# jwr1995/Conv-TasNet

Measured on AMD Instinct MI355X. Metric: utterances/sec (4s, 8kHz, 2-spk) fwd+bwd, higher is better.
Workload: dtype bf16; 1 GPU; paper config train step c2: N=256 L=20 B=256 H=512 P=3 X=8 R=4 gLN non-causal relu-mask, 2 spk, 4 s @ 8 kHz, fwd+PIT loss+bwd+clip+Adam; per_gpu_batch=32, global_batch=32, samples=32000, frames=3199, parallelism=dp1, hip_graph=False

## Files before the change

### conv-tasnet_amd/csrc/ctn_capi.hip

```cpp
#include <stdlib.h>
#include <math.h>
#include <stdarg.h>
#include <stdio.h>
#include <string.h>

#include <atomic>
#include <mutex>
#include <string>
#include <vector>

#include "../../include/ctn.h"
#include "ctn_common.h"
#include "ctn_kernels.h"

using namespace ctn;

static thread_local char g_err[512] = "";

static int fail(int code, const char* fmt, ...) __attribute__((format(printf, 2, 3)));
static int fail(int code, const char* fmt, ...) {
  va_list ap;
  va_start(ap, fmt);
  vsnprintf(g_err, sizeof(g_err), fmt, ap);
  va_end(ap);
// ... 162 lines not shown
  int dev = 0;
  if (hipGetDevice(&dev) != hipSuccess || dev < 0 || dev >= MAX_DEV) return CTN_OK;
  const uint32_t* h = g_deverr.mirror[dev].load(std::memory_order_acquire);
  if (!h) return CTN_OK;
  const uint32_t w = *(const volatile uint32_t*)h;
  if (w) return fail(CTN_ERR_HIP, "device error word 0x%x: %s", w, dev_err_text(w));
  return CTN_OK;
}

hipError_t dev_err_refresh(hipStream_t s) {
  int dev = 0;
  uint32_t* w = dev_err_word(&dev);
  volatile uint32_t* h = w ? dev_err_mirror(dev) : nullptr;
  if (!h) return hipErrorOutOfMemory;
  return hipMemcpyAsync((void*)h, w, 4, hipMemcpyDeviceToHost, s);
}
}

uint32_t* ctn::device_error_word() {
  int dev = 0;
  return dev_err_word(&dev);
}

extern "C" int ctn_device_status(void* stream, uint32_t* word, int clear) {
  int dev = 0;
  uint32_t* dw = dev_err_word(&dev);
  volatile uint32_t* mirror = dw ? dev_err_mirror(dev) : nullptr;
  if (!mirror) return fail(CTN_ERR_HIP, "device error word: unavailable");
  hipStream_t s = (hipStream_t)stream;
  uint32_t w = 0;
// ... 111 lines not shown
  return g;
}
GemmRows tb_gemmB(const ctn_tblock_desc* d, bool fused) {
  GemmRows g{};
  g.g = Rows{d->M, d->K, d->Kp};
  g.Kred = d->H; g.Nout = d->B; g.norm = d->norm_type;
  g.lda = d->H; g.ldw = d->H; g.epi = EPI_RESID; g.ldr = d->B; g.ldc = d->B;
  if (fused) {
    g.aop.kind = OP_NORM1_BWD; g.aop.norm = d->norm_type;
  }
  return g;
}
static int ws_fold_mask() {
  const char* e = getenv("CTN_WS_FOLD");
  return e ? atoi(e) : 3;
}

bool tb_fused_n1(const ctn_tblock_desc* d) {
  const char* e = getenv("CTN_FUSE_N1");
  if (e && atoi(e) == 0) return false;
  if (d->dtype != CTN_DTYPE_BF16 || (d->norm_type != CTN_NORM_GLN && d->norm_type != CTN_NORM_CLN)) return false;
  if (gemm_dual_eligible(BF16, tb_dualB(d))) return false;
  GemmRows g = tb_gemmB(d, true);
  static const float dummy[2] = {0.f, 0.f};
  g.aop.aux = dummy; g.aop.apart = const_cast<float*>(dummy); g.aop.aout = const_cast<float*>(dummy);
  g.aop.stats = reinterpret_cast<const float2*>(dummy); g.aop.sums = reinterpret_cast<const float2*>(dummy);
  return gemm_ws_eligible(BF16, g);
}
DType tb_dt(const ctn_tblock_desc* d) { return d->dtype == CTN_DTYPE_BF16 ? BF16 : F32; }

// ... 324 lines not shown
    w1 = L.w1s;
    w2 = L.w2s;
  }
  GemmRows g1 = tb_gemm1(d);
  g1.A = x;
  g1.W = w1;
  g1.Wf = w1f;
  g1.alpha = p->alpha1;
  g1.C = sv->h1;
  g1.grp_slab = L.slab1;
  const bool fin1 = d->norm_type == CTN_NORM_CLN && gemm_ws_final_cln(dt, g1);
  if (fin1) {
    g1.stats_out = st1;
    g1.eps = (float)kEps;
  }
  {
    TimedScope ts(CTN_TIMER_GEMM1, s);
    CTN_HIP(launch_gemm_rows(dt, g1, s));
  }
  const bool fold = d->norm_type == CTN_NORM_GLN;
  if (!fold && !fin1) CTN_HIP(launch_stats_finalize(L.slab1, G, L.parts1, cnt, 0, (float)kEps, st1, s));
  DwArgs da{};
  da.g = rg; da.H = d->H; da.P = d->P; da.dil = d->dilation; da.pad = tb_pad(d); da.norm = d->norm_type;
  da.seg = dw_seg(da, false);
  da.h1 = sv->h1; da.st1 = st1;
  da.alpha1 = p->alpha1; da.gamma1 = p->gamma1; da.beta1 = p->beta1; da.alpha2 = p->alpha2;
  da.wd = p->wd; da.d_out = sv->d; da.slab2 = L.slab2;
  if (fold) da.f_st1 = gemm_rows_stat_fold(dt, g1, L.slab1, cnt, (float)kEps, 0, st1);
  if (d->norm_type == CTN_NORM_CLN) {
    da.st2_out = st2;
    da.eps = (float)kEps;
  }
  {
    TimedScope ts(CTN_TIMER_DW_FWD, s);
    CTN_HIP(launch_dw_fwd(dt, da, s));
  }
  GemmRows g2{};
  g2.g = rg; g2.Kred = d->H; g2.Nout = d->B; g2.norm = d->norm_type;
  g2.A = sv->d; g2.lda = d->H;
  g2.aop.kind = OP_PRELU_NORM; g2.aop.norm = d->norm_type; g2.aop.stats = st2;
  g2.aop.gamma = p->gamma2; g2.aop.beta = p->beta2; g2.aop.alpha = p->alpha2;
  g2.W = w2; g2.ldw = d->H; g2.Wf = w2f;
  g2.epi = EPI_RESID; g2.R = x; g2.ldr = d->B;
// ... 99 lines not shown
  GemmRows ga = tb_gemmA(d);
  ga.A = gy;
  ga.W = w2t;
  ga.Wf = w2tf;
  ga.R = sv->d;
  ga.alpha = p->alpha2; ga.stats = st2; ga.gamma = p->gamma2;
  ga.C = L.G1;
  ga.grp_slab = L.slabA;
  GemmDual duA = tb_dualA(d);
  duA.A = gy; duA.W = w2t; duA.Wf = w2tf; duA.R = sv->d; duA.C = L.G1;
  duA.alpha = p->alpha2; duA.stats = st2; duA.gamma = p->gamma2; duA.grp_slab = L.slabA;
  duA.Bm = sv->d;
  duA.bop.stats = st2; duA.bop.gamma = p->gamma2; duA.bop.beta = p->beta2; duA.bop.alpha = p->alpha2;
  duA.Dpart = L.cpart2;
  const bool dualA = gemm_dual_eligible(dt, duA);
  if (dualA) {
    TimedScope ts(CTN_TIMER_GEMM_A, s);
    CTN_HIP(launch_gemm_dual(duA, s));
  } else {
    {
      TimedScope ts(CTN_TIMER_GEMM_A, s);
      CTN_HIP(launch_gemm_rows(dt, ga, s));
    }
    GemmCols c2{};
    c2.g = rg; c2.P = d->B; c2.Q = d->H;
    c2.A = gy; c2.lda = d->B;
    c2.B = sv->d; c2.ldb = d->H;
    c2.bop.kind = OP_PRELU_NORM; c2.bop.norm = d->norm_type; c2.bop.stats = st2;
    c2.bop.gamma = p->gamma2; c2.bop.beta = p->beta2; c2.bop.alpha = p->alpha2;
    c2.Cpart = L.cpart2; c2.nchunks = L.chunks2;
    CTN_HIP(launch_gemm_cols(dt, c2, s));
  }
  const bool fold = d->norm_type == CTN_NORM_GLN;

  DwArgs da{};
  da.g = rg; da.H = d->H; da.P = d->P; da.dil = d->dilation; da.pad = tb_pad(d); da.norm = d->norm_type;
  da.seg = dw_seg(da, true);
  da.h1 = sv->h1; da.d = sv->d; da.st1 = st1; da.st2 = st2;
  da.alpha1 = p->alpha1; da.gamma1 = p->gamma1; da.beta1 = p->beta1; da.alpha2 = p->alpha2; da.gamma2 = p->gamma2;
  da.wd = p->wd;
  da.ga2 = L.G1; da.sm2 = L.sums2; da.ga1_out = L.G2; da.slab1 = L.slabD; da.col_slab = L.colD;
  if (fold)
    da.f_sm2 = dualA ? gemm_dual_stat_fold(duA, L.slabA, cnt, 0.f, 1, nullptr)
                     : gemm_rows_stat_fold(dt, ga, L.slabA, cnt, 0.f, 1, nullptr);
  else
    da.sm1_out = L.sums1;
  if (!fold) {
    if (dualA && L.partsA <= 4 && dw_wave_eligible(dt, da))
      da.f_sm2 = gemm_dual_stat_fold(duA, L.slabA, cnt, 0.f, 1, nullptr);
    else
      CTN_HIP(launch_stats_finalize(L.slabA, G, L.partsA, cnt, 1, 0.f, L.sums2, s));
  }
  {
    TimedScope ts(CTN_TIMER_DW_BWD, s);
    CTN_HIP(launch_dw_bwd(dt, da, s));
  }
  const bool fused1 = tb_fused_n1(d);
  int nalpha = ew_blocks(da);
  if (fused1) {
    GemmRows gb = tb_gemmB(d, true);
// ... 1108 lines not shown
```

### conv-tasnet_amd/csrc/ctn_common.h

```cpp
#pragma once
#include <hip/hip_runtime.h>
#include <stdint.h>

#include <type_traits>
#include <utility>

#define CTN_DEV __device__ __forceinline__

typedef uint16_t bf16raw;
struct alignas(16) u128 { uint32_t x, y, z, w; };

CTN_DEV float bf2f(uint16_t v) { return __uint_as_float(((uint32_t)v) << 16); }
CTN_DEV uint16_t f2bf(float f) { return __builtin_bit_cast(uint16_t, (__bf16)f); }

template <typename T> struct Vec8;

template <> struct Vec8<float> {
  static CTN_DEV void load(const float* p, float v[8]) {
    const float4 a = *reinterpret_cast<const float4*>(p);
    const float4 b = *reinterpret_cast<const float4*>(p + 4);
    v[0] = a.x; v[1] = a.y; v[2] = a.z; v[3] = a.w;
    v[4] = b.x; v[5] = b.y; v[6] = b.z; v[7] = b.w;
  }
  static CTN_DEV void store(float* p, const float v[8]) {
// ... 276 lines not shown
}

CTN_DEV float xsum_rows(float v) {
  auto q = __builtin_amdgcn_permlane16_swap(__float_as_uint(v), __float_as_uint(v), false, false);
  v = __uint_as_float(q[0]) + __uint_as_float(q[1]);
  auto r = __builtin_amdgcn_permlane32_swap(__float_as_uint(v), __float_as_uint(v), false, false);
  return __uint_as_float(r[0]) + __uint_as_float(r[1]);
}

template <int CTRL, int ROW_MASK> CTN_DEV double dpp_d(double x) {
  const unsigned long long b = __builtin_bit_cast(unsigned long long, x);
  const unsigned lo = (unsigned)__builtin_amdgcn_update_dpp(0, (int)(unsigned)b, CTRL, ROW_MASK, 0xF, false);
  const unsigned hi = (unsigned)__builtin_amdgcn_update_dpp(0, (int)(unsigned)(b >> 32), CTRL, ROW_MASK, 0xF, false);
  return __builtin_bit_cast(double, ((unsigned long long)hi << 32) | lo);
}
CTN_DEV double wave_sum_dpp_d(double v) {
  v += dpp_d<0xB1, 0xF>(v);
  v += dpp_d<0x4E, 0xF>(v);
  v += dpp_d<0x141, 0xF>(v);
  v += dpp_d<0x140, 0xF>(v);
  v += dpp_d<0x142, 0xA>(v);
  v += dpp_d<0x143, 0xC>(v);
  const unsigned long long b = __builtin_bit_cast(unsigned long long, v);
  const unsigned lo = (unsigned)__builtin_amdgcn_readlane((int)(unsigned)b, 63);
  const unsigned hi = (unsigned)__builtin_amdgcn_readlane((int)(unsigned)(b >> 32), 63);
  return __builtin_bit_cast(double, ((unsigned long long)hi << 32) | lo);
}

#ifndef CTN_IEEE_MAX
#define CTN_IEEE_MAX 0
// ... 48 lines not shown
__host__ __device__ inline int ws_runs_kmax(int ntile, int grid, int tpu) {
  const int twg = (ntile + grid - 1) / grid;
  return (twg + tpu - 1) / tpu + 1;
}

struct StatFold {
  const double2* slab = nullptr;
  int parts = 0;
  double cnt = 1.0;
  float eps = 0.f;
  int mode = 0;
  float2* out = nullptr;
  WsRuns ws;
};

CTN_DEV float2 fold_stat(const StatFold& f, int m) {
  double s = 0.0, ss = 0.0;
  const int lane = (int)(threadIdx.x & 63);
  if (f.ws.grid == 0) {
    const double2* sg = f.slab + (size_t)m * f.parts;
    for (int i = lane; i < f.parts; i += 256) {
      double2 v[4];
#pragma unroll
      for (int u = 0; u < 4; ++u) v[u] = i + 64 * u < f.parts ? sg[i + 64 * u] : make_double2(0.0, 0.0);
#pragma unroll
      for (int u = 0; u < 4; ++u)
        if (i + 64 * u < f.parts) {
          s += v[u].x;
          ss += v[u].y;
        }
    }
// ... 7 lines not shown
      return t0 < ws_t0(w, b + 1) ? f.slab[((size_t)b * w.waves + wv) * w.kmax + (m - t0 / w.tpu)]
                                  : make_double2(0.0, 0.0);
    };
    for (int i = lane; i < n; i += 256) {
      double2 v[4];
#pragma unroll
      for (int u = 0; u < 4; ++u) v[u] = i + 64 * u < n ? get(i + 64 * u) : make_double2(0.0, 0.0);
#pragma unroll
      for (int u = 0; u < 4; ++u)
        if (i + 64 * u < n) {
          s += v[u].x;
          ss += v[u].y;
        }
    }
  }
  s = wave_sum(s);
  ss = wave_sum(ss);
  if (f.mode == 0) {
    const double mean = s / f.cnt;
    double var = ss / f.cnt - mean * mean;
    if (var < 0.0) var = 0.0;
    return make_float2((float)mean, (float)(1.0 / sqrt(var + (double)f.eps)));
  }
  return make_float2((float)(s / f.cnt), (float)(ss / f.cnt));
}

enum NormKind { NORM_GLN = 0, NORM_CLN = 1 };

template <int NK> CTN_DEV int stat_index(int row, int Kp) {
  return NK == NORM_GLN ? row / Kp : row;
}

static inline int ceil_div(long a, long b) { return (int)((a + b - 1) / b); }

template <class F, int... I> CTN_DEV void static_for_impl(F&& f, std::integer_sequence<int, I...>) {
  (f(std::integral_constant<int, I>{}), ...);
}
template <int N, class F> CTN_DEV void static_for(F&& f) { static_for_impl(f, std::make_integer_sequence<int, N>{}); }
```

### conv-tasnet_amd/csrc/ctn_dual_ws.hip

```cpp
#include <stdlib.h>

#include "ctn_common.h"
#include "ctn_kernels.h"

namespace ctn {

namespace {

typedef short bf16x8_t __attribute__((ext_vector_type(8)));
typedef short s16x4_t __attribute__((ext_vector_type(4)));
typedef float f32x4_t __attribute__((ext_vector_type(4)));

constexpr int DV_TM = 32;
#ifndef CTN_DV_NC
#define CTN_DV_NC 8
#endif
constexpr int DV_NR = 4, DV_NC = CTN_DV_NC, DV_NMW = 4;
static_assert(DV_NC == 4 || DV_NC == 8, "column waves");
constexpr int DV_ND = DV_NR + DV_NC;
constexpr int DV_NT = (DV_ND + DV_NMW) * 64;
constexpr int DV_KB = 8, DV_KR = 256;
constexpr int DV_NS = 128;
constexpr int DV_GRID = 256;
#ifndef CTN_DV_RAWB
// ... 167 lines not shown

template <int NK, int NSL, int PF, bool COLS = false>
__global__ __launch_bounds__(COLS ? (DV_NC + DV_NMW) * 64 : DV_NT) void gemm_dual_ws_kernel(GemmDual p) {
  constexpr int NR = COLS ? 0 : DV_NR;
  constexpr int ND = NR + DV_NC;
  constexpr int TM = DV_TM, KB = DV_KB, KR = DV_KR, NS = DV_NS;
  constexpr int SLOT = DV_SLOT;
  static_assert(NSL * SLOT <= 160 * 1024 - 2048, "LDS budget");
  __shared__ __attribute__((aligned(16))) char smem[NSL * SLOT];
  __shared__ __attribute__((aligned(16))) uint32_t fl_full[NSL][4];
  __shared__ __attribute__((aligned(16))) uint32_t fl_done[NSL][ND];
  __shared__ __attribute__((aligned(16))) float sgb[2][NS];
  constexpr bool CLNC = NK == NORM_CLN && !COLS && CTN_DV_CLNC;
  __shared__ __attribute__((aligned(16))) double2 cln_scr[CLNC ? 2 : 1][CLNC ? DV_NR * DV_TM : 1];
  __shared__ __attribute__((aligned(16))) uint32_t fl_rows[2][4];

  const int tid = threadIdx.x, lane = tid & 63, wid = __builtin_amdgcn_readfirstlane(tid >> 6);
  const int lr = lane & 15, lg = lane >> 4;
  const int S = p.Nout / NS;
  const int nr = (int)gridDim.x / S;
  int rr, sl;
  {
    const int b = (int)blockIdx.x;
    if ((int)gridDim.x % (8 * S) == 0) {
      const int l = b / 8;
      sl = l % S;
      rr = (b % 8) * (nr / 8) + l / S;
    } else {
      sl = b % S;
      rr = b / S;
    }
  }
  const long rows = p.g.rows();
  const int ntile = (int)(rows / TM);
  const int t0 = (int)((long)ntile * rr / nr), t1 = (int)((long)ntile * (rr + 1) / nr);
  const int n0 = sl * NS;
  const int Kp = p.g.Kp, Kv = p.g.K, tpu = Kp / TM;

  if (tid < NSL * 4) (&fl_full[0][0])[tid] = 0u;
  else if (tid < NSL * (4 + ND)) (&fl_done[0][0])[tid - NSL * 4] = 0u;
  else if (tid < NSL * (4 + ND) + 8) (&fl_rows[0][0])[tid - NSL * (4 + ND)] = 0u;
  if constexpr (!COLS)
    if (tid < 2 * NS) sgb[tid / NS][tid % NS] = (tid < NS ? p.bop.gamma : p.bop.beta)[n0 + tid % NS];
  __syncthreads();

  const float eal = COLS ? 0.f : p.alpha[0];
  const int kmax = ws_runs_kmax(ntile, nr, tpu);
  constexpr int COLS_LDT = KR + 4;
  static_assert(!COLS || NS * COLS_LDT * 4 <= NSL * DV_SLOT, "transpose image fits the ring");
  static_assert(!COLS || DV_RB, "COLS takes the raw-B slot layout (no operand transform)");
  auto store_tr = [&](float* Dp) __attribute__((always_inline)) {
    const float* img = reinterpret_cast<const float*>(smem);
    for (int idx = tid; idx < NS * (KR / 4); idx += (DV_NC + DV_NMW) * 64) {
      const int nl = idx / (KR / 4), k4 = idx % (KR / 4);
      *reinterpret_cast<float4*>(Dp + (size_t)(n0 + nl) * KR + 4 * k4) =
          *reinterpret_cast<const float4*>(img + nl * COLS_LDT + 4 * k4);
// ... 165 lines not shown
                p.grp_slab[((size_t)t * TM + 16 * rb + lr) * (S * DV_NR) + sl * DV_NR + r] = make_double2((double)s, (double)ss);
            }
          }
        }
        dv_signal(&fl_done[slot][r], gen);
        if (++slot == NSL) {
          slot = 0;
          ++gen;
        }
      }
      DV_ACC(3, tl0);
    };
    if (t0 < t1) {
      if (eal <= 1.f) run(std::true_type{});
      else run(std::false_type{});
      if constexpr (NK == NORM_GLN) flush();
    }
    DV_STAMP_STORE;
    return;
  }
  if (wid < ND) {
    dv_prio<2, NK>();
    constexpr int CJ = COLS ? DV_CJC : (DV_NI ? CTN_DV_CJN : DV_CJ), CI = 16 * (8 / CJ) / DV_NC;
    static_assert(CI >= 2 && CI <= 16 && CI % 2 == 0, "column split");
    const int c = wid - NR, wp = c / (8 / CJ), wn = c % (8 / CJ);
    DV_STAMP_DECL;
    f32x4_t dacc[CI][CJ];
#pragma unroll
    for (int i = 0; i < CI; ++i)
#pragma unroll
      for (int j = 0; j < CJ; ++j) dacc[i][j] = f32x4_t{0.f, 0.f, 0.f, 0.f};
// ... 355 lines not shown
```

### conv-tasnet_amd/csrc/ctn_dw_wave.hip

```cpp
#include <stdlib.h>

#include "ctn_common.h"
#include "ctn_dw.h"
#include "ctn_kernels.h"

namespace ctn {

namespace {

constexpr int WV_H = 512, WV_P = 3, WV_NB = 3;

struct WItem {
  int m, wgi, rho, j0, j1, base;
};
CTN_DEV WItem witem(const DwArgs& a, const CombGeom& gm) {
  const int wv = __builtin_amdgcn_readfirstlane((int)(threadIdx.x >> 6));
  WItem it;
  it.m = (int)blockIdx.x / gm.wgpu;
  it.wgi = (int)blockIdx.x % gm.wgpu;
  const int id = it.wgi * gm.ipw + wv;
  const bool active = id < gm.items;
  it.rho = active ? id / gm.nseg : 0;
  it.j0 = active ? (id % gm.nseg) * a.seg : 0;
  it.j1 = active ? min(it.j0 + a.seg, gm.jmax) : it.j0;
// ... 24 lines not shown

template <int NK, bool CAUSAL>
__global__ __launch_bounds__(256, 4) void dw_fwd_wave_kernel(DwArgs a) {
  constexpr int P = WV_P, H = WV_H;
  constexpr int POWN = CAUSAL ? P - 1 : (P - 1) / 2;
  constexpr int HT = P - 1 - POWN;
  __shared__ double red[16];
  const CombGeom gm = comb_geom(a);
  const WItem it = witem(a, gm);
  const int lane = threadIdx.x & 63;
  const int K = a.g.K, Kp = a.g.Kp, dil = a.dil;
  const long nbytes = a.g.rows() * H * 2;
  const rsrc_t rH = du_rsrc(a.h1, nbytes);
  const uint32_t vo = lane * 16;
  const float al1 = a.alpha1[0], al2 = a.alpha2[0];
  float2 st1u = make_float2(0.f, 0.f);
  if constexpr (NK == NORM_GLN) {
    const StatFold& f = a.f_st1;
    if (f.slab) {
      st1u = fold_stat(f, it.m);
      if (f.out && it.wgi == 0 && threadIdx.x == 0) f.out[it.m] = st1u;
    } else {
      st1u = a.st1[it.m];
    }
    st1u = uniform2(st1u);
  }
  float w[P][8], g1[8], b1[8];
#pragma unroll
  for (int e = 0; e < 8; ++e) {
    const int ch = lane * 8 + e;
    g1[e] = a.gamma1[ch];
    b1[e] = a.beta1[ch];
#pragma unroll
    for (int t = 0; t < P; ++t) w[t][e] = a.wd[ch * P + t];
  }
  const int jK = steps_below(K, it.rho, dil);
  auto row_at = [&](int s) { return it.base + ((unsigned)s < (unsigned)jK ? it.rho + s * dil : 0); };
  auto ld = [&](int row) {
    return __builtin_bit_cast(v4u, __builtin_amdgcn_raw_buffer_load_b128(rH, vo, row * (H * 2), (CTN_DW_NTL & 2) ? 2 : 0));
  };

  constexpr int CB = 63;
  float2 bst = make_float2(0.f, 0.f), nst = bst;
  int bbase = it.j0;
  auto batch_fetch = [&](int jb) { nst = a.st1[row_at(jb + lane + HT)]; };
  auto batch_next = [&]() {
    bbase += CB;
    bst = nst;
    batch_fetch(bbase + CB);
  };
  auto bcast = [&](float2 v, int j) {
    const int l = j - bbase;
    return make_float2(__int_as_float(__builtin_amdgcn_readlane(__float_as_int(v.x), l)),
                       __int_as_float(__builtin_amdgcn_readlane(__float_as_int(v.y), l)));
  };
// ... 2 lines not shown
    float x[8];
    unpack8(vh, x);
    const float nm = -st.x;
#pragma unroll
    for (int e = 0; e < 8; ++e) {
      const float ax = x[e] * al1;
      const float v = fmaf((sel_pos(x[e], x[e], ax) + nm) * st.y, g1[e], b1[e]);
      out[e] = EDGE ? (ok ? v : 0.f) : v;
    }
  };
  float win[3][8];
#pragma unroll
  for (int i = 0; i < P - 1; ++i) {
    const int sh = it.j0 - POWN + i;
    const int rh = row_at(sh);
    finish(std::true_type{}, ld(rh), (unsigned)sh < (unsigned)jK, NK == NORM_GLN ? st1u : a.st1[rh], win[i + 1]);
  }

  float ts = 0.f, tss = 0.f;
  RowPark pk;
  pk.j0 = it.j0;
  auto park_flush = [&](int n) {
    const int k = it.rho + (pk.j0 + lane) * dil;
    if (lane < n && k < Kp) {
      if (a.st2_out) {
        const double mean = (double)pk.s / H;
        double var = (double)pk.ss / H - mean * mean;
        if (var < 0.0) var = 0.0;
        a.st2_out[it.base + k] = make_float2((float)mean, (float)(1.0 / sqrt(var + (double)a.eps)));
      } else {
        a.slab2[it.base + k] = make_double2((double)pk.s, (double)pk.ss);
// ... 30 lines not shown
    } else {
      s = wave_sum_dpp(s);
      ss = wave_sum_dpp(ss);
      const int pq = j - pk.j0;
      pk.s = lane == pq ? s : pk.s;
      pk.ss = lane == pq ? ss : pk.ss;
    }
  };
  auto boundary = [&]() {
    park_flush(CB);
    pk.j0 = bbase + CB;
    batch_next();
  };

  const int jint = min(it.j1, jK - HT);
  v4u rb[WV_NB];
  if (it.j0 < it.j1) rb[0] = ld(row_at(it.j0 + HT));
  if (it.j0 + 1 < it.j1) rb[1] = ld(row_at(it.j0 + 1 + HT));
  if constexpr (NK != NORM_GLN) {
    batch_fetch(it.j0);
    bbase = it.j0 - CB;
    batch_next();
  }
  auto triple = [&](int jb) __attribute__((always_inline)) {
    static_for<3>([&](auto qc) __attribute__((always_inline)) {
      constexpr int q = decltype(qc)::value;
      const int j = jb + q;
      __builtin_amdgcn_sched_barrier(0);
      rb[(q + 2) % 3] = ld(row_at(j + 2 + HT));
      step(std::false_type{}, qc, j, rb[q]);
    });
  };
  int jb = it.j0;
// ... 40 lines not shown
  constexpr int GT = POWN;
  __shared__ double red[16];
  __shared__ float buf[256 * 8];
  const CombGeom gm = comb_geom(a);
  const WItem it = witem(a, gm);
  const int lane = threadIdx.x & 63;
  const int K = a.g.K, Kp = a.g.Kp, dil = a.dil;
  const long nbytes = a.g.rows() * H * 2;
  const rsrc_t rH = du_rsrc(a.h1, nbytes), rD = du_rsrc(a.d, nbytes), rG = du_rsrc(a.ga2, nbytes);
  const uint32_t vo = lane * 16;
  const float al1 = a.alpha1[0], al2 = a.alpha2[0];
  float2 st1u = make_float2(0.f, 0.f), st2u = st1u, sm2u = st1u;
  if constexpr (NK == NORM_GLN) {
    st1u = a.st1[it.m];
    st2u = a.st2[it.m];
    const StatFold& f = a.f_sm2;
    sm2u = f.slab ? fold_stat(f, it.m) : a.sm2[it.m];
    sm2u = uniform2(sm2u);
  }
  __shared__ __attribute__((aligned(16))) float cst[P + 3][H];
  for (int i = threadIdx.x; i < H; i += 256) {
    const int c = CTN_DW_CSTH ? ((i >> 2) & 1) * (H / 2) + (i >> 3) * 4 + (i & 3) : i;
#pragma unroll
    for (int t = 0; t < P; ++t) cst[t][c] = a.wd[i * P + t];
    cst[P][c] = a.gamma1[i];
    cst[P + 1][c] = a.beta1[i];
    cst[P + 2][c] = a.gamma2[i];
  }
  __syncthreads();
  auto cbase = [&]() __attribute__((always_inline)) {
    uint32_t b = lane * (CTN_DW_CSTH ? 16u : 32u);
    asm volatile("" : "+v"(b));
    return b;
  };
  auto cvec4 = [&](uint32_t b, int r, int hf) __attribute__((always_inline)) {
    return *reinterpret_cast<const float4*>(reinterpret_cast<const char*>(&cst[0][0]) + b + (r * H * 4 + hf * (CTN_DW_CSTH ? H * 2 : 16)));
  };
  auto f4 = [](const float4& v, int i) { return i == 0 ? v.x : i == 1 ? v.y : i == 2 ? v.z : v.w; };
  float cgam[8], cbet[8], cgam2[8], cbet2[8], cwd[P][8];
#pragma unroll
  for (int e = 0; e < 8; ++e) {
    cgam[e] = cbet[e] = cgam2[e] = cbet2[e] = 0.f;
#pragma unroll
    for (int t = 0; t < P; ++t) cwd[t][e] = 0.f;
// ... 98 lines not shown
    }
  };
  auto gstat = [&](int row, int j, bool batch, float2& st, float2& sm) __attribute__((always_inline)) {
    if constexpr (NK == NORM_GLN) {
      st = st2u;
      sm = sm2u;
    } else if (batch) {
      st = bcast(bst2, j);
      sm = bcast(bsm2, j);
    } else {
      st = a.st2[row];
      sm = sm_row(row);
    }
  };

#pragma unroll
  for (int i = 0; i < P - 1; ++i) {
    const int sg = it.j0 + GT - P + 1 + i;
    const int rg = row_at(sg);
    float2 st, sm;
    gstat(rg, 0, false, st, sm);
    finish_g(std::true_type{}, ld(rD, rg), ld(rG, rg), sg >= 0 && sg < jK, sg >= it.j0 && sg < it.j1, st, sm,
             gdw[i + 1]);
  }

  RowPark pk;
  pk.j0 = it.j0;
  auto park_flush = [&](int n) {
    const int k = it.rho + (pk.j0 + lane) * dil;
    if (lane < n && k < Kp) {
      if (a.sm1_out)
        a.sm1_out[it.base + k] = make_float2((float)((double)pk.s / H), (float)((double)pk.ss / H));
      else
        a.slab1[it.base + k] = make_double2((double)pk.s, (double)pk.ss);
    }
  };

// ... 55 lines not shown
    } else {
      s = wave_sum_dpp(s);
      ss = wave_sum_dpp(ss);
      const int pq = j - pk.j0;
      pk.s = lane == pq ? s : pk.s;
      pk.ss = lane == pq ? ss : pk.ss;
    }
  };
  auto boundary = [&]() {
    park_flush(CB);
    pk.j0 = bbase + CB;
    batch_next();
  };

  const int jint = min(it.j1, jK) - GT;
  BwdRow rb[WV_NB];
  if (it.j0 < it.j1) load_row(it.j0, rb[0]);
  if (it.j0 + 1 < it.j1) load_row(it.j0 + 1, rb[1]);
  if constexpr (NK != NORM_GLN) {
    batch_fetch(it.j0);
    bbase = it.j0 - CB;
    batch_next();
  }
  auto triple = [&](int jb) __attribute__((always_inline)) {
    static_for<3>([&](auto qc) __attribute__((always_inline)) {
      constexpr int q = decltype(qc)::value;
      const int j = jb + q;
      __builtin_amdgcn_sched_barrier(0);
      load_row(j + 2, rb[(q + 2) % 3]);
      step(std::false_type{}, qc, j, rb[q]);
    });
  };
  int jb = it.j0;
// ... 97 lines not shown
```

### conv-tasnet_amd/csrc/ctn_gemm_ws.hip

```cpp
#include <stdlib.h>

#include <type_traits>

#include "ctn_common.h"
#include "ctn_kernels.h"

namespace ctn {

typedef short bf16x8_t __attribute__((ext_vector_type(8)));
typedef float f32x4_t __attribute__((ext_vector_type(4)));

#ifndef CTN_WS_GRID
#define CTN_WS_GRID 256
#endif
constexpr int WS_WAVES = 8, WS_TM = 16, WS_GRID = CTN_WS_GRID;
#ifndef CTN_WS_DMA
#define CTN_WS_DMA 1
#endif
#ifndef CTN_WS_DR
#define CTN_WS_DR 6
#endif
constexpr int WS_DR = CTN_WS_DR;
#ifndef CTN_WS_FLAGS
#define CTN_WS_FLAGS 0
// ... 676 lines not shown
      if (t < t1) {
        step(t, accC, accP);
        epilogue(le1, t1 - 1, accC);
      } else {
        epilogue(le1, t1 - 1, accP);
      }
    }
  };
  const float al_any = (OPK == OP_PRELU_NORM || N1B) ? oal : eal;
  if constexpr (OPK == OP_PRELU_NORM || N1B || HAS_STATS) {
    if (al_any <= 1.f) run(std::true_type{});
    else run(std::false_type{});
  } else {
    run(std::true_type{});
  }
  if constexpr (HAS_STATS && NK == NORM_GLN) flush_run();
  if constexpr (CLN_FIN) {
    lds_barrier();
    cln_final(t1 - 1);
  }
#if CTN_WS_STAMP
  if (lane == 0)
    for (int i = 0; i < 8; ++i) ws_stamps[((size_t)blockIdx.x * 16 + wid) * 8 + i] = st_sum[i];
#endif
  if constexpr (N1B) {
    const float w = wave_sum_dpp(calpha);
    if (lane == 0) salpha[wid] = w;
    __syncthreads();
    if (tid == 0) {
      double a = 0.0;
      for (int i = 0; i < WV; ++i) a += (double)salpha[i];
// ... 94 lines not shown
static int ws_waves(const GemmRows& p) { return ws_wide(p) ? 16 * (p.Nout / 512) : 8; }
static int ws_tile_rows(const GemmRows& p) { return ws_wide(p) ? 32 : WS_TM; }
static int ws_slices(const GemmRows& p) { return p.Nout == 1536 ? 3 : ws_wide(p) ? CTN_WS_S512 : 1; }

template <int OPK, int NK, int EPI>
static hipError_t ws_launch_shape(const GemmRows& p, hipStream_t s) {
  int nb = 0, kb = 0;
  ws_shape(p.Nout, p.Kred, &nb, &kb);
  const dim3 grid(gemm_ws_grid(p));
  if (nb == 4 && kb == 8) {
    if constexpr (EPI == EPI_NORM_BWD)
      hipLaunchKernelGGL((gemm_ws_kernel<OPK, NK, EPI, 4, 8, 8, 1>), grid, dim3(512), 0, s, p);
    else if (ws_slices(p) == 3) {
      if constexpr (OPK == OP_PLAIN && EPI == EPI_STORE)
        hipLaunchKernelGGL((gemm_ws_kernel<OPK, NK, EPI, 2, 8, 16, 2, 3>), grid, dim3(1024), 0, s, p);
    } else if (ws_slices(p) == 2)
      hipLaunchKernelGGL((gemm_ws_kernel<OPK, NK, EPI, 2, 8, 8, 2, 2>), grid, dim3(512), 0, s, p);
    else
      hipLaunchKernelGGL((gemm_ws_kernel<OPK, NK, EPI, 2, 8, 16, 2>), grid, dim3(1024), 0, s, p);
  }
  else if (nb == 2 && kb == 16)
    hipLaunchKernelGGL((gemm_ws_kernel<OPK, NK, EPI, 2, 16, 8, 1>), grid, dim3(512), 0, s, p);
  else
    hipLaunchKernelGGL((gemm_ws_kernel<OPK, NK, EPI, 2, 8, 8, 1>), grid, dim3(512), 0, s, p);
  return hipGetLastError();
}

template <int NK>
static hipError_t ws_launch_nk(const GemmRows& p, hipStream_t s) {
  if (p.aop.kind == OP_PRELU_NORM) return ws_launch_shape<OP_PRELU_NORM, NK, EPI_RESID>(p, s);
// ... 19 lines not shown
```

### conv-tasnet_amd/csrc/ctn_kernels.h

```cpp
#pragma once
#include <hip/hip_runtime.h>
#include <stddef.h>
#include <stdint.h>

#include "ctn_common.h"

namespace ctn {

enum DType { F32 = 0, BF16 = 1 };

uint32_t* device_error_word();
enum RowOpKind { OP_PLAIN = 0, OP_NORM = 1, OP_PRELU_NORM = 2, OP_NORM1_BWD = 3 };
enum EpiKind { EPI_STORE = 0, EPI_PRELU_STATS = 1, EPI_RESID = 2, EPI_NORM_BWD = 3 };

struct RowOp {
  int kind = OP_PLAIN;
  int norm = 0;
  const float2* stats = nullptr;
  const float* gamma = nullptr;
  const float* beta = nullptr;
  const float* alpha = nullptr;
  StatFold fold;
  const void* aux = nullptr;
  const float2* sums = nullptr;
// ... 12 lines not shown
  const void* A; int lda;
  const void* W; int ldw;
  const void* Wf;
  RowOp aop;
  int epi = EPI_STORE;
  void* C; int ldc;
  const void* R = nullptr; int ldr = 0;
  const float* alpha = nullptr;
  const float2* stats = nullptr;
  const float* gamma = nullptr;
  int norm = 0;
  double2* grp_slab = nullptr;
  float2* stats_out = nullptr;
  float eps = 0.f;
  uint32_t* err = nullptr;
};
int gemm_rows_tiles_per_group(DType dt, const GemmRows& p);
hipError_t launch_gemm_rows(DType dt, const GemmRows& p, hipStream_t s);
bool gemm_ws_eligible(DType dt, const GemmRows& p);
int gemm_ws_grid(const GemmRows& p);
int gemm_ws_group_parts(const GemmRows& p);
WsRuns gemm_ws_runs(const GemmRows& p);
StatFold gemm_rows_stat_fold(DType dt, const GemmRows& p, const double2* slab, double cnt, float eps, int mode,
                             float2* out);
bool gemm_ws_can_fold(DType dt, const GemmRows& p);
bool gemm_ws_final_cln(DType dt, const GemmRows& p);
hipError_t launch_gemm_ws(const GemmRows& p, hipStream_t s);

struct GemmCols {
  Rows g;
// ... 12 lines not shown
  const void* A; int lda;
  const void* W; int ldw;
  const void* Wf;
  int epi = EPI_RESID;
  void* C; int ldc;
  const void* R = nullptr; int ldr = 0;
  const float* alpha = nullptr;
  const float2* stats = nullptr;
  const float* gamma = nullptr;
  int norm = 0;
  double2* grp_slab = nullptr;
  const void* Bm; int ldb;
  RowOp bop;
  float* Dpart;
  uint32_t* err = nullptr;
};
bool gemm_dual_eligible(DType dt, const GemmDual& p);
int gemm_dual_ranges(const GemmDual& p);
int gemm_dual_group_parts(const GemmDual& p);
int dual_ws_cln_parts_per_slice();
int dual_ws_row_waves(const GemmDual& p);
StatFold gemm_dual_stat_fold(const GemmDual& p, const double2* slab, double cnt, float eps, int mode,
                             float2* out);
hipError_t launch_gemm_dual(const GemmDual& p, hipStream_t s);
bool gemm_dual_ws_enabled();
bool gemm_dual_ws_eligible(const GemmDual& p);
int gemm_dual_ws_ranges(const GemmDual& p);
hipError_t launch_gemm_dual_ws(const GemmDual& p, hipStream_t s);
bool gemm_cols_ws_eligible(DType dt, const GemmCols& c);
int gemm_cols_ws_ranges(const GemmCols& c);
// ... 190 lines not shown
```

Baseline: 2401 utterances/sec.

## Add opt-in ticketed in-GEMM stat finalization and prefetch dw rows before stat fold

Result: no change. 2420 utterances/sec, median of 6 (+0.8%).

```diff
diff --git a/conv-tasnet_amd/csrc/ctn_capi.hip b/conv-tasnet_amd/csrc/ctn_capi.hip
--- a/conv-tasnet_amd/csrc/ctn_capi.hip
+++ b/conv-tasnet_amd/csrc/ctn_capi.hip
@@ -200,6 +200,34 @@
   volatile uint32_t* h = w ? dev_err_mirror(dev) : nullptr;
   if (!h) return hipErrorOutOfMemory;
   return hipMemcpyAsync((void*)h, w, 4, hipMemcpyDeviceToHost, s);
+}
+}
+
+constexpr uint32_t STAT_TICKETS = 1u << 15;
+__device__ uint32_t ctn_stat_ticket_words[STAT_TICKETS];
+
+namespace {
+struct StatTickets {
+  std::atomic<uint32_t*> base[MAX_DEV] = {};
+  std::atomic<uint32_t> next[MAX_DEV] = {};
+};
+StatTickets g_tickets;
+
+uint32_t* stat_tickets(int n) {
+  int dev = 0;
+  if (n < 1 || (uint32_t)n > STAT_TICKETS / 8) return nullptr;
+  if (hipGetDevice(&dev) != hipSuccess || dev < 0 || dev >= MAX_DEV) return nullptr;
+  uint32_t* b = g_tickets.base[dev].load(std::memory_order_acquire);
+  if (!b) {
+    void* a = nullptr;
+    if (hipGetSymbolAddress(&a, HIP_SYMBOL(ctn_stat_ticket_words)) != hipSuccess) return nullptr;
+    b = (uint32_t*)a;
+    g_tickets.base[dev].store(b, std::memory_order_release);
+  }
+  uint32_t o = g_tickets.next[dev].load(std::memory_order_relaxed), start;
+  do start = o + (uint32_t)n > STAT_TICKETS ? 0u : o;
+  while (!g_tickets.next[dev].compare_exchange_weak(o, start + (uint32_t)n, std::memory_order_relaxed));
+  return b + start;
 }
 }
 
@@ -341,6 +369,11 @@
 static int ws_fold_mask() {
   const char* e = getenv("CTN_WS_FOLD");
   return e ? atoi(e) : 3;
+}
+
+static bool stat_final_enabled() {
+  const char* e = getenv("CTN_STAT_FINAL");
+  return e && atoi(e) != 0;
 }
 
 bool tb_fused_n1(const ctn_tblock_desc* d) {
@@ -695,11 +728,18 @@
     g1.stats_out = st1;
     g1.eps = (float)kEps;
   }
+  const bool fold = d->norm_type == CTN_NORM_GLN;
+  bool final1 = false;
+  if (fold && stat_final_enabled() && gemm_ws_eligible(dt, g1)) {
+    g1.fin.f = gemm_rows_stat_fold(dt, g1, L.slab1, cnt, (float)kEps, 0, st1);
+    g1.fin.per_range = gemm_ws_grid(g1) / g1.fin.f.ws.grid;
+    g1.fin.ticket = stat_tickets(G);
+    final1 = g1.fin.ticket != nullptr;
+  }
   {
     TimedScope ts(CTN_TIMER_GEMM1, s);
     CTN_HIP(launch_gemm_rows(dt, g1, s));
   }
-  const bool fold = d->norm_type == CTN_NORM_GLN;
   if (!fold && !fin1) CTN_HIP(launch_stats_finalize(L.slab1, G, L.parts1, cnt, 0, (float)kEps, st1, s));
   DwArgs da{};
   da.g = rg; da.H = d->H; da.P = d->P; da.dil = d->dilation; da.pad = tb_pad(d); da.norm = d->norm_type;
@@ -707,7 +747,7 @@
   da.h1 = sv->h1; da.st1 = st1;
   da.alpha1 = p->alpha1; da.gamma1 = p->gamma1; da.beta1 = p->beta1; da.alpha2 = p->alpha2;
   da.wd = p->wd; da.d_out = sv->d; da.slab2 = L.slab2;
-  if (fold) da.f_st1 = gemm_rows_stat_fold(dt, g1, L.slab1, cnt, (float)kEps, 0, st1);
+  if (fold && !final1) da.f_st1 = gemm_rows_stat_fold(dt, g1, L.slab1, cnt, (float)kEps, 0, st1);
   if (d->norm_type == CTN_NORM_CLN) {
     da.st2_out = st2;
     da.eps = (float)kEps;
@@ -837,6 +877,13 @@
   duA.bop.stats = st2; duA.bop.gamma = p->gamma2; duA.bop.beta = p->beta2; duA.bop.alpha = p->alpha2;
   duA.Dpart = L.cpart2;
   const bool dualA = gemm_dual_eligible(dt, duA);
+  bool final2 = false;
+  if (dualA && d->norm_type == CTN_NORM_GLN && stat_final_enabled() && gemm_dual_ws_eligible(duA)) {
+    duA.fin.f = gemm_dual_stat_fold(duA, L.slabA, cnt, 0.f, 1, L.sums2);
+    duA.fin.per_range = duA.fin.f.ws.waves / dual_ws_row_waves(duA);
+    duA.fin.ticket = stat_tickets(G);
+    final2 = duA.fin.ticket != nullptr;
+  }
   if (dualA) {
     TimedScope ts(CTN_TIMER_GEMM_A, s);
     CTN_HIP(launch_gemm_dual(duA, s));
@@ -863,10 +910,10 @@
   da.alpha1 = p->alpha1; da.gamma1 = p->gamma1; da.beta1 = p->beta1; da.alpha2 = p->alpha2; da.gamma2 = p->gamma2;
   da.wd = p->wd;
   da.ga2 = L.G1; da.sm2 = L.sums2; da.ga1_out = L.G2; da.slab1 = L.slabD; da.col_slab = L.colD;
-  if (fold)
+  if (fold && !final2)
     da.f_sm2 = dualA ? gemm_dual_stat_fold(duA, L.slabA, cnt, 0.f, 1, nullptr)
                      : gemm_rows_stat_fold(dt, ga, L.slabA, cnt, 0.f, 1, nullptr);
-  else
+  else if (!fold)
     da.sm1_out = L.sums1;
   if (!fold) {
     if (dualA && L.partsA <= 4 && dw_wave_eligible(dt, da))
diff --git a/conv-tasnet_amd/csrc/ctn_common.h b/conv-tasnet_amd/csrc/ctn_common.h
--- a/conv-tasnet_amd/csrc/ctn_common.h
+++ b/conv-tasnet_amd/csrc/ctn_common.h
@@ -314,6 +314,23 @@
   const unsigned hi = (unsigned)__builtin_amdgcn_update_dpp(0, (int)(unsigned)(b >> 32), CTRL, ROW_MASK, 0xF, false);
   return __builtin_bit_cast(double, ((unsigned long long)hi << 32) | lo);
 }
+template <bool W32> CTN_DEV double swap_sum_d(double v) {
+  const unsigned long long b = __builtin_bit_cast(unsigned long long, v);
+  const unsigned lo = (unsigned)b, hi = (unsigned)(b >> 32);
+  auto ql = W32 ? __builtin_amdgcn_permlane32_swap(lo, lo, false, false) : __builtin_amdgcn_permlane16_swap(lo, lo, false, false);
+  auto qh = W32 ? __builtin_amdgcn_permlane32_swap(hi, hi, false, false) : __builtin_amdgcn_permlane16_swap(hi, hi, false, false);
+  return __builtin_bit_cast(double, ((unsigned long long)qh[0] << 32) | ql[0]) +
+         __builtin_bit_cast(double, ((unsigned long long)qh[1] << 32) | ql[1]);
+}
+CTN_DEV double wave_sum_xor_valu_d(double v) {
+  v = swap_sum_d<true>(v);
+  v = swap_sum_d<false>(v);
+  v += dpp_d<0x128, 0xF>(v);
+  v += dpp_d<0x1B, 0xF>(dpp_d<0x141, 0xF>(v));
+  v += dpp_d<0x4E, 0xF>(v);
+  v += dpp_d<0xB1, 0xF>(v);
+  return v;
+}
 CTN_DEV double wave_sum_dpp_d(double v) {
   v += dpp_d<0xB1, 0xF>(v);
   v += dpp_d<0x4E, 0xF>(v);
@@ -392,7 +409,7 @@
   WsRuns ws;
 };
 
-CTN_DEV float2 fold_stat(const StatFold& f, int m) {
+template <bool VALU = false> CTN_DEV float2 fold_stat(const StatFold& f, int m) {
   double s = 0.0, ss = 0.0;
   const int lane = (int)(threadIdx.x & 63);
   if (f.ws.grid == 0) {
@@ -430,8 +447,8 @@
         }
     }
   }
-  s = wave_sum(s);
-  ss = wave_sum(ss);
+  s = VALU ? wave_sum_xor_valu_d(s) : wave_sum(s);
+  ss = VALU ? wave_sum_xor_valu_d(ss) : wave_sum(ss);
   if (f.mode == 0) {
     const double mean = s / f.cnt;
     double var = ss / f.cnt - mean * mean;
@@ -441,6 +458,42 @@
   return make_float2((float)(s / f.cnt), (float)(ss / f.cnt));
 }
 
+struct StatFinal {
+  uint32_t* ticket = nullptr;
+  int per_range = 1;
+  StatFold f;
+};
+__host__ __device__ inline uint32_t ws_tickets_of(const StatFinal& sf, int m) {
+  const WsRuns& w = sf.f.ws;
+  const int blo = ws_block_of_tile(w, m * w.tpu), bhi = ws_block_of_tile(w, (m + 1) * w.tpu - 1);
+  int n = 0;
+  for (int b = blo; b <= bhi; ++b) n += ws_t0(w, b) < ws_t0(w, b + 1);
+  return (uint32_t)(n * sf.per_range);
+}
+CTN_DEV void stat_final_wave(const StatFinal& sf, int mlo, int mhi) {
+  const int lane = (int)(threadIdx.x & 63);
+  __builtin_amdgcn_fence(__ATOMIC_RELEASE, "agent");
+  for (int base = mlo; base <= mhi; base += 64) {
+    const int m = base + lane;
+    bool last = false;
+    if (m <= mhi)
+      last = __hip_atomic_fetch_add(sf.ticket + m, 1u, __ATOMIC_RELAXED, __HIP_MEMORY_SCOPE_AGENT) + 1u ==
+             ws_tickets_of(sf, m);
+    unsigned long long todo = __ballot(last);
+    if (!todo) continue;
+    __builtin_amdgcn_fence(__ATOMIC_ACQUIRE, "agent");
+    while (todo) {
+      const int mi = base + __builtin_ctzll(todo);
+      todo &= todo - 1;
+      const float2 v = fold_stat<true>(sf.f, mi);
+      if (lane == 0) {
+        sf.f.out[mi] = v;
+        __hip_atomic_store(sf.ticket + mi, 0u, __ATOMIC_RELAXED, __HIP_MEMORY_SCOPE_AGENT);
+      }
+    }
+  }
+}
+
 enum NormKind { NORM_GLN = 0, NORM_CLN = 1 };
 
 template <int NK> CTN_DEV int stat_index(int row, int Kp) {
diff --git a/conv-tasnet_amd/csrc/ctn_dual_ws.hip b/conv-tasnet_amd/csrc/ctn_dual_ws.hip
--- a/conv-tasnet_amd/csrc/ctn_dual_ws.hip
+++ b/conv-tasnet_amd/csrc/ctn_dual_ws.hip
@@ -205,6 +205,7 @@
   constexpr bool CLNC = NK == NORM_CLN && !COLS && CTN_DV_CLNC;
   __shared__ __attribute__((aligned(16))) double2 cln_scr[CLNC ? 2 : 1][CLNC ? DV_NR * DV_TM : 1];
   __shared__ __attribute__((aligned(16))) uint32_t fl_rows[2][4];
+  __shared__ uint32_t fin_rows;
 
   const int tid = threadIdx.x, lane = tid & 63, wid = __builtin_amdgcn_readfirstlane(tid >> 6);
   const int lr = lane & 15, lg = lane >> 4;
@@ -231,6 +232,7 @@
   if (tid < NSL * 4) (&fl_full[0][0])[tid] = 0u;
   else if (tid < NSL * (4 + ND)) (&fl_done[0][0])[tid - NSL * 4] = 0u;
   else if (tid < NSL * (4 + ND) + 8) (&fl_rows[0][0])[tid - NSL * (4 + ND)] = 0u;
+  else if (tid == NSL * (4 + ND) + 8) fin_rows = 0u;
   if constexpr (!COLS)
     if (tid < 2 * NS) sgb[tid / NS][tid % NS] = (tid < NS ? p.bop.gamma : p.bop.beta)[n0 + tid % NS];
   __syncthreads();
@@ -426,7 +428,14 @@
     if (t0 < t1) {
       if (eal <= 1.f) run(std::true_type{});
       else run(std::false_type{});
-      if constexpr (NK == NORM_GLN) flush();
+      if constexpr (NK == NORM_GLN) {
+        flush();
+        if (p.fin.ticket) {
+          uint32_t nth = 0;
+          if (lane == 0) nth = __hip_atomic_fetch_add(&fin_rows, 1u, __ATOMIC_ACQ_REL, __HIP_MEMORY_SCOPE_WORKGROUP);
+          if (__builtin_amdgcn_readfirstlane((int)nth) == NR - 1) stat_final_wave(p.fin, m0, run_m);
+        }
+      }
     }
     DV_STAMP_STORE;
     return;
diff --git a/conv-tasnet_amd/csrc/ctn_dw_wave.hip b/conv-tasnet_amd/csrc/ctn_dw_wave.hip
--- a/conv-tasnet_amd/csrc/ctn_dw_wave.hip
+++ b/conv-tasnet_amd/csrc/ctn_dw_wave.hip
@@ -62,6 +62,25 @@
   const rsrc_t rH = du_rsrc(a.h1, nbytes);
   const uint32_t vo = lane * 16;
   const float al1 = a.alpha1[0], al2 = a.alpha2[0];
+  float w[P][8], g1[8], b1[8];
+#pragma unroll
+  for (int e = 0; e < 8; ++e) {
+    const int ch = lane * 8 + e;
+    g1[e] = a.gamma1[ch];
+    b1[e] = a.beta1[ch];
+#pragma unroll
+    for (int t = 0; t < P; ++t) w[t][e] = a.wd[ch * P + t];
+  }
+  const int jK = steps_below(K, it.rho, dil);
+  auto row_at = [&](int s) { return it.base + ((unsigned)s < (unsigned)jK ? it.rho + s * dil : 0); };
+  auto ld = [&](int row) {
+    return __builtin_bit_cast(v4u, __builtin_amdgcn_raw_buffer_load_b128(rH, vo, row * (H * 2), (CTN_DW_NTL & 2) ? 2 : 0));
+  };
+  v4u pro[P - 1], rb[WV_NB];
+#pragma unroll
+  for (int i = 0; i < P - 1; ++i) pro[i] = ld(row_at(it.j0 - POWN + i));
+  if (it.j0 < it.j1) rb[0] = ld(row_at(it.j0 + HT));
+  if (it.j0 + 1 < it.j1) rb[1] = ld(row_at(it.j0 + 1 + HT));
   float2 st1u = make_float2(0.f, 0.f);
   if constexpr (NK == NORM_GLN) {
     const StatFold& f = a.f_st1;
@@ -73,20 +92,6 @@
     }
     st1u = uniform2(st1u);
   }
-  float w[P][8], g1[8], b1[8];
-#pragma unroll
-  for (int e = 0; e < 8; ++e) {
-    const int ch = lane * 8 + e;
-    g1[e] = a.gamma1[ch];
-    b1[e] = a.beta1[ch];
-#pragma unroll
-    for (int t = 0; t < P; ++t) w[t][e] = a.wd[ch * P + t];
-  }
-  const int jK = steps_below(K, it.rho, dil);
-  auto row_at = [&](int s) { return it.base + ((unsigned)s < (unsigned)jK ? it.rho + s * dil : 0); };
-  auto ld = [&](int row) {
-    return __builtin_bit_cast(v4u, __builtin_amdgcn_raw_buffer_load_b128(rH, vo, row * (H * 2), (CTN_DW_NTL & 2) ? 2 : 0));
-  };
 
   constexpr int CB = 63;
   float2 bst = make_float2(0.f, 0.f), nst = bst;
@@ -119,7 +124,7 @@
   for (int i = 0; i < P - 1; ++i) {
     const int sh = it.j0 - POWN + i;
     const int rh = row_at(sh);
-    finish(std::true_type{}, ld(rh), (unsigned)sh < (unsigned)jK, NK == NORM_GLN ? st1u : a.st1[rh], win[i + 1]);
+    finish(std::true_type{}, pro[i], (unsigned)sh < (unsigned)jK, NK == NORM_GLN ? st1u : a.st1[rh], win[i + 1]);
   }
 
   float ts = 0.f, tss = 0.f;
@@ -180,9 +185,6 @@
   };
 
   const int jint = min(it.j1, jK - HT);
-  v4u rb[WV_NB];
-  if (it.j0 < it.j1) rb[0] = ld(row_at(it.j0 + HT));
-  if (it.j0 + 1 < it.j1) rb[1] = ld(row_at(it.j0 + 1 + HT));
   if constexpr (NK != NORM_GLN) {
     batch_fetch(it.j0);
     bbase = it.j0 - CB;
@@ -253,20 +255,29 @@
   if constexpr (NK == NORM_GLN) {
     st1u = a.st1[it.m];
     st2u = a.st2[it.m];
-    const StatFold& f = a.f_sm2;
-    sm2u = f.slab ? fold_stat(f, it.m) : a.sm2[it.m];
-    sm2u = uniform2(sm2u);
   }
   __shared__ __attribute__((aligned(16))) float cst[P + 3][H];
-  for (int i = threadIdx.x; i < H; i += 256) {
-    const int c = CTN_DW_CSTH ? ((i >> 2) & 1) * (H / 2) + (i >> 3) * 4 + (i & 3) : i;
-#pragma unroll
-    for (int t = 0; t < P; ++t) cst[t][c] = a.wd[i * P + t];
-    cst[P][c] = a.gamma1[i];
-    cst[P + 1][c] = a.beta1[i];
-    cst[P + 2][c] = a.gamma2[i];
-  }
-  __syncthreads();
+  static_assert(H % 256 == 0, "whole rounds of the 256 threads");
+  float cstv[H / 256][P + 3];
+#pragma unroll
+  for (int u = 0; u < H / 256; ++u) {
+    const int i = (int)threadIdx.x + 256 * u;
+#pragma unroll
+    for (int t = 0; t < P; ++t) cstv[u][t] = a.wd[i * P + t];
+    cstv[u][P] = a.gamma1[i];
+    cstv[u][P + 1] = a.beta1[i];
+    cstv[u][P + 2] = a.gamma2[i];
+  }
+  auto stage_cst = [&]() __attribute__((always_inline)) {
+#pragma unroll
+    for (int u = 0; u < H / 256; ++u) {
+      const int i = (int)threadIdx.x + 256 * u;
+      const int c = CTN_DW_CSTH ? ((i >> 2) & 1) * (H / 2) + (i >> 3) * 4 + (i & 3) : i;
+#pragma unroll
+      for (int t = 0; t < P + 3; ++t) cst[t][c] = cstv[u][t];
+    }
+    __syncthreads();
+  };
   auto cbase = [&]() __attribute__((always_inline)) {
     uint32_t b = lane * (CTN_DW_CSTH ? 16u : 32u);
     asm volatile("" : "+v"(b));
@@ -395,13 +406,29 @@
     }
   };
 
+  v4u prd[P - 1], prg[P - 1];
+#pragma unroll
+  for (int i = 0; i < P - 1; ++i) {
+    const int rg = row_at(it.j0 + GT - P + 1 + i);
+    prd[i] = ld(rD, rg);
+    prg[i] = ld(rG, rg);
+  }
+  BwdRow rb[WV_NB];
+  if (it.j0 < it.j1) load_row(it.j0, rb[0]);
+  if (it.j0 + 1 < it.j1) load_row(it.j0 + 1, rb[1]);
+  if constexpr (NK == NORM_GLN) {
+    const StatFold& f = a.f_sm2;
+    sm2u = f.slab ? fold_stat(f, it.m) : a.sm2[it.m];
+    sm2u = uniform2(sm2u);
+  }
+  stage_cst();
 #pragma unroll
   for (int i = 0; i < P - 1; ++i) {
     const int sg = it.j0 + GT - P + 1 + i;
     const int rg = row_at(sg);
     float2 st, sm;
     gstat(rg, 0, false, st, sm);
-    finish_g(std::true_type{}, ld(rD, rg), ld(rG, rg), sg >= 0 && sg < jK, sg >= it.j0 && sg < it.j1, st, sm,
+    finish_g(std::true_type{}, prd[i], prg[i], sg >= 0 && sg < jK, sg >= it.j0 && sg < it.j1, st, sm,
              gdw[i + 1]);
   }
 
@@ -487,9 +514,6 @@
   };
 
   const int jint = min(it.j1, jK) - GT;
-  BwdRow rb[WV_NB];
-  if (it.j0 < it.j1) load_row(it.j0, rb[0]);
-  if (it.j0 + 1 < it.j1) load_row(it.j0 + 1, rb[1]);
   if constexpr (NK != NORM_GLN) {
     batch_fetch(it.j0);
     bbase = it.j0 - CB;
diff --git a/conv-tasnet_amd/csrc/ctn_gemm_ws.hip b/conv-tasnet_amd/csrc/ctn_gemm_ws.hip
--- a/conv-tasnet_amd/csrc/ctn_gemm_ws.hip
+++ b/conv-tasnet_amd/csrc/ctn_gemm_ws.hip
@@ -714,7 +714,13 @@
   } else {
     run(std::true_type{});
   }
-  if constexpr (HAS_STATS && NK == NORM_GLN) flush_run();
+  if constexpr (HAS_STATS && NK == NORM_GLN) {
+    flush_run();
+    if (p.fin.ticket) {
+      __syncthreads();
+      if (wid == 0) stat_final_wave(p.fin, m0, run_m);
+    }
+  }
   if constexpr (CLN_FIN) {
     lds_barrier();
     cln_final(t1 - 1);
@@ -839,6 +845,8 @@
     else if (ws_slices(p) == 3) {
       if constexpr (OPK == OP_PLAIN && EPI == EPI_STORE)
         hipLaunchKernelGGL((gemm_ws_kernel<OPK, NK, EPI, 2, 8, 16, 2, 3>), grid, dim3(1024), 0, s, p);
+      else
+        return hipErrorInvalidValue;
     } else if (ws_slices(p) == 2)
       hipLaunchKernelGGL((gemm_ws_kernel<OPK, NK, EPI, 2, 8, 8, 2, 2>), grid, dim3(512), 0, s, p);
     else
diff --git a/conv-tasnet_amd/csrc/ctn_kernels.h b/conv-tasnet_amd/csrc/ctn_kernels.h
--- a/conv-tasnet_amd/csrc/ctn_kernels.h
+++ b/conv-tasnet_amd/csrc/ctn_kernels.h
@@ -50,6 +50,7 @@
   float2* stats_out = nullptr;
   float eps = 0.f;
   uint32_t* err = nullptr;
+  StatFinal fin;
 };
 int gemm_rows_tiles_per_group(DType dt, const GemmRows& p);
 hipError_t launch_gemm_rows(DType dt, const GemmRows& p, hipStream_t s);
@@ -92,6 +93,7 @@
   RowOp bop;
   float* Dpart;
   uint32_t* err = nullptr;
+  StatFinal fin;
 };
 bool gemm_dual_eligible(DType dt, const GemmDual& p);
 int gemm_dual_ranges(const GemmDual& p);
```
